# jake3991/sonar-SLAM

Measured on AMD Instinct MI355X. Metric: keyframes/sec (CFAR+ICP) on 512x1024 sonar, 5k-pt pairs, higher is better.
Workload: dtype u8 (CFAR, integer-exact) + f32/f64-accumulate (ICP); 1 GPU; BASELINE configs[1]: 4096 keyframes/step/GPU = 1024x512 SOCA-CFAR(Ntc40,Ngc10)+gate65 -> remap+nonzero+px2m -> downsample 0.5 -> remove_outlier 1.0/5 -> 5000x5000-pt ICP (p2plane30); batch_per_gpu=4096, distinct_frames=256, screened_out_pings=0, icp_mode=p2plane30, parallelism=job farm x1, icp_prep_stream=side, batches_in_flight=1, icp_converged_jobs=4096, max_points_per_frame=17494, points_capacity=32768, full=False

## Files before the change

### include/sonarfe.h

```cpp
#ifndef SONARFE_H
#define SONARFE_H

#include <stddef.h>
#include <stdint.h>

#ifdef __cplusplus
extern "C" {
#endif

typedef struct sfe_ctx sfe_ctx;
typedef struct sfe_geom sfe_geom;

#define SFE_ERR_ARG (-1)
#define SFE_ERR_HIP (-2)
#define SFE_ERR_NODEV (-3)
#define SFE_ERR_CAP (-4)

#define SFE_CFAR_CA 0
#define SFE_CFAR_SOCA 1
#define SFE_CFAR_GOCA 2
#define SFE_CFAR_OS 3

#define SFE_ICP_OK 0
#define SFE_ICP_NO_OUTLIER 1
// ... 119 lines not shown
int sfe_icp_compute_pairs_chain(sfe_ctx *ctx, const sfe_icp_params *p, const sfe_icp_dpf *rd, int n_rd,
                                const sfe_icp_dpf *rf, int n_rf, const float *src, const int32_t *src_off, const float *tgt,
                                const int32_t *tgt_off, const float *guesses9, int n_jobs, float *T_out9, int32_t *status,
                                int32_t *iters);
int sfe_icp_compute_jobs_chain(sfe_ctx *ctx, const sfe_icp_params *p, const sfe_icp_dpf *rd, int n_rd,
                               const sfe_icp_dpf *rf, int n_rf, const float *src, int n_src_pts, const float *tgt,
                               int n_tgt_pts, const int32_t *jobs4, const float *guesses9, int n_jobs, float *T_out9,
                               int32_t *status, int32_t *iters);
typedef struct sfe_icp_outliers {
    int use_min_dist;
    float min_dist;
    int use_median;
    float median_factor;
    int use_bound;
    float max_rotation_norm;
    float max_translation_norm;
    int bound_order;
} sfe_icp_outliers;
int sfe_icp_compute_guesses_chain_ext(sfe_ctx *ctx, const sfe_icp_params *p, const sfe_icp_outliers *o,
                                      const sfe_icp_dpf *rd, int n_rd, const sfe_icp_dpf *rf, int n_rf, const float *src,
                                      int n_src, const float *tgt, int n_tgt, const float *guesses9, int n_guesses,
                                      float *T_out9, int32_t *status, int32_t *iters);
int sfe_icp_compute_pairs_chain_ext(sfe_ctx *ctx, const sfe_icp_params *p, const sfe_icp_outliers *o,
                                    const sfe_icp_dpf *rd, int n_rd, const sfe_icp_dpf *rf, int n_rf, const float *src,
                                    const int32_t *src_off, const float *tgt, const int32_t *tgt_off, const float *guesses9,
                                    int n_jobs, float *T_out9, int32_t *status, int32_t *iters);
int sfe_icp_compute_jobs_chain_ext(sfe_ctx *ctx, const sfe_icp_params *p, const sfe_icp_outliers *o,
                                   const sfe_icp_dpf *rd, int n_rd, const sfe_icp_dpf *rf, int n_rf, const float *src,
                                   int n_src_pts, const float *tgt, int n_tgt_pts, const int32_t *jobs4, const float *guesses9,
                                   int n_jobs, float *T_out9, int32_t *status, int32_t *iters);
int sfe_icp_set_tuning(sfe_ctx *ctx, int variant);
int sfe_icp_get_profile(sfe_ctx *ctx, int enable, long long *cycles16);
#define SFE_ICP_ROUTE_TINY 0
#define SFE_ICP_ROUTE_T0 1
#define SFE_ICP_ROUTE_T1 2
#define SFE_ICP_ROUTE_Q 3
#define SFE_ICP_ROUTE_LDS 4
#define SFE_ICP_ROUTE_GLB 5
#define SFE_ICP_ROUTE_SPLIT 6
#define SFE_ICP_ROUTE_BRUTE 7
int sfe_icp_last_routes(sfe_ctx *ctx, int32_t *route, int n_jobs, int32_t *n_cu);
int sfe_icp_batch_dev(sfe_ctx *ctx, const sfe_icp_params *p, const float *d_src,
                      const int32_t *src_off, const float *d_tgt, const int32_t *tgt_off,
                      const float *d_guess9, int n_jobs, float *d_T9, int32_t *d_status,
                      int32_t *d_iters);

int sfe_icp_jobs_dev(sfe_ctx *ctx, const sfe_icp_params *p, const float *d_src, const float *d_tgt,
                     const int32_t *jobs4, const float *d_guess9, int n_jobs, float *d_T9, int32_t *d_status,
                     int32_t *d_iters);

int sfe_cloud_filter_batch_dev(sfe_ctx *ctx, const double *d_pts, const int32_t *d_counts, int n_frames,
                               int64_t cap, float resolution, double radius, int min_points,
                               float *d_out, int32_t *d_out_counts);
int sfe_cloud_filter_staged_dev(sfe_ctx *ctx, int n_frames, int64_t cap, float resolution, double radius,
                                int min_points, float *d_out, int32_t *d_out_counts);

int sfe_feature_extract_ping(sfe_ctx *ctx, sfe_geom *g, const uint8_t *img, int alg, int train_hs, int guard_hs,
                             int k, double tau, int intensity_thr, float resolution, double radius, int min_points,
                             int64_t cap, float *cloud_out, int32_t *n_out, int32_t *n_raw_out, uint8_t *vis_out);

typedef struct sfe_cloud_store sfe_cloud_store;
#define SFE_STORE_NEGATE_Y 1
#define SFE_PING_VIS_JET 4
#define SFE_STORE_F32_POINTS 2
int sfe_cloud_store_create(sfe_ctx *ctx, int64_t capacity_points, int32_t max_clouds, sfe_cloud_store **out);
void sfe_cloud_store_destroy(sfe_cloud_store *s);
int sfe_cloud_store_count(sfe_cloud_store *s);
int sfe_cloud_store_put(sfe_ctx *ctx, sfe_cloud_store *s, int64_t stamp, const float *pts, int n, int32_t *handle_out);
int sfe_cloud_store_put_batch_dev(sfe_ctx *ctx, sfe_cloud_store *s, const int64_t *stamps, const float *d_clouds,
                                  const int32_t *d_counts, int n_frames, int64_t cap, int flags, int32_t *handles_out);
int sfe_cloud_store_meta(sfe_ctx *ctx, sfe_cloud_store *s, int32_t first, int32_t n, int64_t *stamps, int64_t *offsets,
                         int32_t *counts);
int sfe_cloud_store_read(sfe_ctx *ctx, sfe_cloud_store *s, int32_t handle, float *out, int cap, int *n_out);
int sfe_cloud_store_truncate(sfe_ctx *ctx, sfe_cloud_store *s, int32_t n_slots);
int sfe_cloud_store_get_points(sfe_ctx *ctx, sfe_cloud_store *s, const int32_t *handles, const float *T6, int n_jobs, int m,
                               float resolution, int flags, const int64_t *stamps, int32_t *handles_out);
int sfe_icp_store_jobs_dev(sfe_ctx *ctx, const sfe_icp_params *p, sfe_cloud_store *s, const int32_t *pairs,
                           const float *d_guess9, int n_jobs, float *d_T9, int32_t *d_status, int32_t *d_iters);
int sfe_icp_store_compute(sfe_ctx *ctx, const sfe_icp_params *p, sfe_cloud_store *s, const int32_t *pairs,
                          const float *guesses9, int n_jobs, float *T_out9, int32_t *status, int32_t *iters);
int sfe_icp_store_compute_chain_ext(sfe_ctx *ctx, const sfe_icp_params *p, const sfe_icp_outliers *o,
                                    const sfe_icp_dpf *rd, int n_rd, const sfe_icp_dpf *rf, int n_rf,
                                    sfe_cloud_store *s, const int32_t *pairs, const float *guesses9, int n_jobs,
                                    float *T_out9, int32_t *status, int32_t *iters);
int sfe_cloud_store_overlap(sfe_ctx *ctx, sfe_cloud_store *s, const int32_t *pairs, const float *T6, int n_jobs,
                            float max_dist, int flags, int32_t *counts_out);
int sfe_cloud_store_get_points_keys(sfe_ctx *ctx, sfe_cloud_store *s, const int32_t *handles, const float *T6,
                                    const int32_t *keys, int m, float resolution, int flags, int64_t stamp, int32_t *handle_out);
int sfe_cloud_store_read_keys(sfe_ctx *ctx, sfe_cloud_store *s, int32_t handle, int32_t *out, int cap, int *n_out);
int sfe_cloud_store_fov_select(sfe_ctx *ctx, sfe_cloud_store *s, int32_t handle, const float *Tinv6, const double *range_bound,
                               const double *bearing_bound, int n_frames, int n_keys, int32_t *key_counts_out,
                               int32_t *n_selected_out, int32_t *n_ambiguous_out);
int sfe_cloud_store_set_selection(sfe_ctx *ctx, sfe_cloud_store *s, int32_t handle, const uint8_t *sel, int n);
int sfe_cloud_store_compact_selected(sfe_ctx *ctx, sfe_cloud_store *s, int32_t handle, int64_t stamp, int32_t *handle_out);
int sfe_cloud_store_match_keys(sfe_ctx *ctx, sfe_cloud_store *s, int32_t source, const float *T6, int32_t target, float max_dist,
                               int flags, int n_keys, int32_t *key_counts_out, int32_t *overlap_out);
int sfe_cloud_store_get_points_keys_many(sfe_ctx *ctx, sfe_cloud_store *s, const int32_t *handles, const float *T6,
                                         const int32_t *keys, const int32_t *job_off, int n_jobs, float resolution, int flags,
                                         const int64_t *stamps, int32_t *handles_out);
int sfe_cloud_store_fov_select_many(sfe_ctx *ctx, sfe_cloud_store *s, const int32_t *handles, int n_jobs, const float *Tinv6,
                                    const double *range_bound, const double *bearing_bound, const int32_t *frame_off,
                                    int n_keys, int32_t *key_counts_out, int32_t *n_selected_out, int32_t *n_ambiguous_out);
int sfe_cloud_store_compact_selected_many(sfe_ctx *ctx, sfe_cloud_store *s, const int32_t *handles, int n_jobs,
                                          const int64_t *stamps, int32_t *handles_out);
int sfe_cloud_store_match_keys_many(sfe_ctx *ctx, sfe_cloud_store *s, const int32_t *sources, const float *T6,
                                    const int32_t *targets, int n_jobs, float max_dist, int flags, int n_keys,
// ... 64 lines not shown
```

### sonar_slam_amd/_lib.py

```python
import contextlib
import ctypes as C
import os
import threading

import numpy as np

_HERE = os.path.dirname(os.path.abspath(__file__))
LIB_PATH = os.environ.get("SONARFE_LIB") or os.path.join(_HERE, "libsonarfe.so")

SFE_ERR_CAP = -4

ICP_ROUTE_TINY = 0
ICP_ROUTE_T0 = 1
ICP_ROUTE_T1 = 2
ICP_ROUTE_Q = 3
ICP_ROUTE_LDS = 4
ICP_ROUTE_GLB = 5
ICP_ROUTE_SPLIT = 6
ICP_ROUTE_BRUTE = 7

ALG = {"CA": 0, "SOCA": 1, "GOCA": 2, "OS": 3}

ICP_STATUS_MESSAGES = {
    0: "success",
# ... 124 lines not shown
    "sfe_geom_destroy": (None, [_vp]),
    "sfe_remap_u8": (C.c_int, [_vp, _vp, _u8p, _u8p]),
    "sfe_remap_u8_dev": (C.c_int, [_vp, _vp, _vp, _vp]),
    "sfe_colormap_lut": (C.c_int, [C.c_int, _u8p]),
    "sfe_remap_u8_colormap": (C.c_int, [_vp, _vp, _u8p, C.c_int, _u8p]),
    "sfe_remap_u8_colormap_dev": (C.c_int, [_vp, _vp, _vp, C.c_int, _vp]),
    "sfe_feature_extract_ping": (C.c_int, [_vp, _vp, _u8p, C.c_int, C.c_int, C.c_int, C.c_int, C.c_double, C.c_int, C.c_float,
                                           C.c_double, C.c_int, C.c_int64, _f32p, _i32p, _i32p, _u8p]),
    "sfe_extract_points": (C.c_int, [_vp, _vp, _u8p, C.c_int64, _i64p, _f64p, _i64p]),
    "sfe_extract_set_tuning": (C.c_int, [_vp, C.c_int]),
    "sfe_extract_points_batch_dev": (C.c_int, [_vp, _vp, _vp, C.c_int, C.c_int64, _vp, _vp]),
    "sfe_extract_points_bits_batch_dev": (C.c_int, [_vp, _vp, _vp, C.c_int, C.c_int64, _vp, _vp]),
    "sfe_extract_points_bits_staged_dev": (C.c_int, [_vp, _vp, _vp, C.c_int, C.c_int64, _vp, C.c_int, _vp]),
    "sfe_match": (C.c_int, [_vp, _f32p, C.c_int, _f32p, C.c_int, C.c_float, _i32p, _f32p]),
    "sfe_match_knn": (C.c_int, [_vp, _f32p, C.c_int, _f32p, C.c_int, C.c_int, C.c_float, _i32p, _f32p]),
    "sfe_knn_density": (C.c_int, [_vp, _f32p, C.c_int, C.c_int, _f32p]),
    "sfe_remove_outlier": (C.c_int, [_vp, _f32p, C.c_int, C.c_double, C.c_int, _f32p,
                                     C.POINTER(C.c_int)]),
    "sfe_downsample": (C.c_int, [_vp, _f32p, C.c_int, C.c_float, _f32p, _i32p, C.POINTER(C.c_int)]),
    "sfe_icp_compute": (C.c_int, [_vp, C.POINTER(IcpParams), _f32p, C.c_int, _f32p, C.c_int, _f32p,
                                  _f32p, C.POINTER(C.c_int)]),
    "sfe_icp_compute_guesses": (C.c_int, [_vp, C.POINTER(IcpParams), _f32p, C.c_int, _f32p, C.c_int,
                                          _f32p, C.c_int, _f32p, _i32p, _i32p]),
    "sfe_icp_compute_pairs": (C.c_int, [_vp, C.POINTER(IcpParams), _f32p, _i32p, _f32p, _i32p, _f32p, C.c_int,
                                        _f32p, _i32p, _i32p]),
    "sfe_icp_compute_jobs": (C.c_int, [_vp, C.POINTER(IcpParams), _f32p, C.c_int, _f32p, C.c_int, _i32p, _f32p, C.c_int,
                                       _f32p, _i32p, _i32p]),
    "sfe_icp_filter_clouds_dev": (C.c_int, [_vp, C.POINTER(IcpDpf), C.c_int, _vp, _i32p, C.c_int, _vp, _i32p]),
    "sfe_icp_compute_guesses_chain": (C.c_int, [_vp, C.POINTER(IcpParams), C.POINTER(IcpDpf), C.c_int, C.POINTER(IcpDpf),
                                                C.c_int, _f32p, C.c_int, _f32p, C.c_int, _f32p, C.c_int, _f32p, _i32p, _i32p]),
    "sfe_icp_compute_pairs_chain": (C.c_int, [_vp, C.POINTER(IcpParams), C.POINTER(IcpDpf), C.c_int, C.POINTER(IcpDpf),
                                              C.c_int, _f32p, _i32p, _f32p, _i32p, _f32p, C.c_int, _f32p, _i32p, _i32p]),
    "sfe_icp_compute_jobs_chain": (C.c_int, [_vp, C.POINTER(IcpParams), C.POINTER(IcpDpf), C.c_int, C.POINTER(IcpDpf),
                                             C.c_int, _f32p, C.c_int, _f32p, C.c_int, _i32p, _f32p, C.c_int, _f32p, _i32p,
                                             _i32p]),
    "sfe_icp_compute_guesses_chain_ext": (C.c_int, [_vp, C.POINTER(IcpParams), C.POINTER(IcpOutliers), C.POINTER(IcpDpf),
                                                    C.c_int, C.POINTER(IcpDpf), C.c_int, _f32p, C.c_int, _f32p, C.c_int,
                                                    _f32p, C.c_int, _f32p, _i32p, _i32p]),
    "sfe_icp_compute_pairs_chain_ext": (C.c_int, [_vp, C.POINTER(IcpParams), C.POINTER(IcpOutliers), C.POINTER(IcpDpf),
                                                  C.c_int, C.POINTER(IcpDpf), C.c_int, _f32p, _i32p, _f32p, _i32p, _f32p,
                                                  C.c_int, _f32p, _i32p, _i32p]),
    "sfe_icp_compute_jobs_chain_ext": (C.c_int, [_vp, C.POINTER(IcpParams), C.POINTER(IcpOutliers), C.POINTER(IcpDpf),
                                                 C.c_int, C.POINTER(IcpDpf), C.c_int, _f32p, C.c_int, _f32p, C.c_int, _i32p,
                                                 _f32p, C.c_int, _f32p, _i32p, _i32p]),
    "sfe_icp_set_tuning": (C.c_int, [_vp, C.c_int]),
    "sfe_icp_get_profile": (C.c_int, [_vp, C.c_int, C.POINTER(C.c_longlong)]),
    "sfe_icp_last_routes": (C.c_int, [_vp, _i32p, C.c_int, _i32p]),
    "sfe_icp_batch_dev": (C.c_int, [_vp, C.POINTER(IcpParams), _vp, _i32p, _vp, _i32p, _vp, C.c_int,
                                    _vp, _vp, _vp]),
    "sfe_icp_jobs_dev": (C.c_int, [_vp, C.POINTER(IcpParams), _vp, _vp, _i32p, _vp, C.c_int, _vp, _vp, _vp]),
    "sfe_cloud_filter_batch_dev": (C.c_int, [_vp, _vp, _vp, C.c_int, C.c_int64, C.c_float, C.c_double, C.c_int,
                                             _vp, _vp]),
    "sfe_cloud_filter_staged_dev": (C.c_int, [_vp, C.c_int, C.c_int64, C.c_float, C.c_double, C.c_int, _vp, _vp]),
    "sfe_cloud_store_create": (C.c_int, [_vp, C.c_int64, C.c_int32, C.POINTER(_vp)]),
    "sfe_cloud_store_destroy": (None, [_vp]),
    "sfe_cloud_store_count": (C.c_int, [_vp]),
    "sfe_cloud_store_put": (C.c_int, [_vp, _vp, C.c_int64, _f32p, C.c_int, _i32p]),
    "sfe_cloud_store_put_batch_dev": (C.c_int, [_vp, _vp, _i64p, _vp, _vp, C.c_int, C.c_int64, C.c_int, _i32p]),
    "sfe_cloud_store_meta": (C.c_int, [_vp, _vp, C.c_int32, C.c_int32, _i64p, _i64p, _i32p]),
    "sfe_cloud_store_read": (C.c_int, [_vp, _vp, C.c_int32, _f32p, C.c_int, C.POINTER(C.c_int)]),
    "sfe_cloud_store_truncate": (C.c_int, [_vp, _vp, C.c_int32]),
    "sfe_cloud_store_get_points": (C.c_int, [_vp, _vp, _i32p, _f32p, C.c_int, C.c_int, C.c_float, C.c_int, _i64p, _i32p]),
    "sfe_icp_store_jobs_dev": (C.c_int, [_vp, C.POINTER(IcpParams), _vp, _i32p, _vp, C.c_int, _vp, _vp, _vp]),
    "sfe_icp_store_compute": (C.c_int, [_vp, C.POINTER(IcpParams), _vp, _i32p, _f32p, C.c_int, _f32p, _i32p, _i32p]),
    "sfe_icp_store_compute_chain_ext": (C.c_int, [_vp, C.POINTER(IcpParams), C.POINTER(IcpOutliers), C.POINTER(IcpDpf),
                                                  C.c_int, C.POINTER(IcpDpf), C.c_int, _vp, _i32p, _f32p, C.c_int, _f32p,
                                                  _i32p, _i32p]),
    "sfe_cloud_store_overlap": (C.c_int, [_vp, _vp, _i32p, _f32p, C.c_int, C.c_float, C.c_int, _i32p]),
    "sfe_feature_extract_ping_store": (C.c_int, [_vp, _vp, _vp, C.c_int64, _u8p, C.c_int, C.c_int, C.c_int, C.c_int,
                                                 C.c_double, C.c_int, C.c_float, C.c_double, C.c_int, C.c_int64, C.c_int,
                                                 _i32p, _i32p, _i32p, _f32p, _u8p]),
    "sfe_costgrid_create": (C.c_int, [_vp, _i32p, _i32p, C.c_int, C.c_int, C.c_int, C.c_int, C.POINTER(_vp)]),
    "sfe_costgrid_destroy": (None, [_vp]),
    "sfe_costgrid_download": (C.c_int, [_vp, _vp, C.c_int, _u8p]),
    "sfe_matching_cost_batch": (C.c_int, [_vp, _vp, _f32p, C.c_int, _f32p, C.c_int, C.c_float, C.c_float,
                                          C.c_double, C.c_int, _i32p]),
    "sfe_costgrid_create_store": (C.c_int, [_vp, _vp, _i32p, C.c_int, _f32p, _f32p, C.c_float, _i32p, _i32p, C.c_int,
                                            C.POINTER(_vp)]),
    "sfe_matching_cost_store": (C.c_int, [_vp, _vp, _vp, _i32p, _i32p, C.c_int, _f32p, C.c_int, C.c_double, C.c_int, _i32p]),
    "sfe_shgo_sobol_replay": (C.c_int, [C.c_int, _i32p, _i32p, _f64p, _i32p, C.c_int, _u8p, _i32p, _i32p, _i32p]),
    "sfe_matching_cost_store_samples": (C.c_int, [_vp, _vp, _vp, _i32p, _i32p, C.c_int, _f64p, _f64p, _f64p, C.c_int, C.c_double, C.c_int,
                                                  _i32p]),
    "sfe_pose2_sample_transforms": (C.c_int, [_f64p, _f64p, C.c_int, _f64p, C.c_int, _f32p]),
    "sfe_cloud_store_bbox": (C.c_int, [_vp, _vp, _i32p, C.c_int, _f32p]),
    "sfe_cloud_store_get_points_keys": (C.c_int, [_vp, _vp, _i32p, _f32p, _i32p, C.c_int, C.c_float, C.c_int, C.c_int64, _i32p]),
    "sfe_cloud_store_read_keys": (C.c_int, [_vp, _vp, C.c_int32, _i32p, C.c_int, C.POINTER(C.c_int)]),
    "sfe_cloud_store_fov_select": (C.c_int, [_vp, _vp, C.c_int32, _f32p, _f64p, _f64p, C.c_int, C.c_int, _i32p, _i32p, _i32p]),
    "sfe_cloud_store_set_selection": (C.c_int, [_vp, _vp, C.c_int32, _u8p, C.c_int]),
    "sfe_cloud_store_compact_selected": (C.c_int, [_vp, _vp, C.c_int32, C.c_int64, _i32p]),
    "sfe_cloud_store_match_keys": (C.c_int, [_vp, _vp, C.c_int32, _f32p, C.c_int32, C.c_float, C.c_int, C.c_int, _i32p, _i32p]),
    "sfe_cloud_store_get_points_keys_many": (C.c_int, [_vp, _vp, _i32p, _f32p, _i32p, _i32p, C.c_int, C.c_float, C.c_int, _i64p,
                                                       _i32p]),
    "sfe_cloud_store_fov_select_many": (C.c_int, [_vp, _vp, _i32p, C.c_int, _f32p, _f64p, _f64p, _i32p, C.c_int, _i32p, _i32p,
                                                  _i32p]),
    "sfe_cloud_store_compact_selected_many": (C.c_int, [_vp, _vp, _i32p, C.c_int, _i64p, _i32p]),
    "sfe_cloud_store_match_keys_many": (C.c_int, [_vp, _vp, _i32p, _f32p, _i32p, C.c_int, C.c_float, C.c_int, C.c_int, _i32p,
                                                  _i32p]),
    "sfe_map_create": (C.c_int, [_vp, C.c_int, C.c_int, C.POINTER(_vp)]),
    "sfe_map_destroy": (None, [_vp]),
    "sfe_map_geometry": (C.c_int, [_vp, _f32p, C.c_int, C.c_int, C.POINTER(C.c_int)]),
    "sfe_map_set_logodds": (C.c_int, [_vp, C.c_int, C.c_int, _f32p]),
    "sfe_map_measure": (C.c_int, [_vp, C.c_int, _i32p, _i32p, _i32p, _i32p, _i32p, _i32p, _f32p, C.c_int, _f64p,
                                  C.c_float, C.c_float, C.c_float, C.c_float]),
    "sfe_map_measure_stages": (C.c_int, [_vp, C.c_int, _u8p, _f32p, _i32p]),
    "sfe_map_fit_bounds": (C.c_int, [_vp, C.c_int, _i32p, _f64p, _f64p, C.c_double, _i32p]),
    "sfe_map_grow": (C.c_int, [_vp, C.c_int, C.c_int, C.c_int, C.c_int]),
# ... 195 lines not shown
```

### sonar_slam_amd/csrc/sfe_cloudfilter.hip

```cpp
#include "sfe_cloudfilter.h"

#include <algorithm>
#include <cstdio>
#include <cstdlib>

__global__ __launch_bounds__(1024) void cf_cast_bbox_kernel(const double *__restrict__ pts64,
                                                            const int32_t *__restrict__ counts, long long cap,
                                                            float max_size, float2 *__restrict__ p32,
                                                            CfHeader *__restrict__ hdrs)
{
    __shared__ float s_mn[2][16], s_mx[2][16];
    const int f = blockIdx.x;
    const int n = (int)min((long long)max(counts[f], 0), cap);
    const double *src = pts64 + (size_t)f * cap * 2;
    float2 *dst = p32 + (size_t)f * cap;
    float mnx = INFINITY, mny = INFINITY, mxx = -INFINITY, mxy = -INFINITY;
    for (int i = threadIdx.x; i < n; i += 1024) {
        const float2 p = make_float2((float)src[2 * i], (float)src[2 * i + 1]);
        dst[i] = p;
        mnx = fminf(mnx, p.x);
        mxx = fmaxf(mxx, p.x);
        mny = fminf(mny, p.y);
        mxy = fmaxf(mxy, p.y);
    }
#pragma unroll
    for (int d = 32; d >= 1; d >>= 1) {
        mnx = fminf(mnx, __shfl_down(mnx, d));
        mxx = fmaxf(mxx, __shfl_down(mxx, d));
        mny = fminf(mny, __shfl_down(mny, d));
        mxy = fmaxf(mxy, __shfl_down(mxy, d));
    }
    if ((threadIdx.x & 63) == 0) {
        s_mn[0][threadIdx.x >> 6] = mnx;
        s_mn[1][threadIdx.x >> 6] = mny;
        s_mx[0][threadIdx.x >> 6] = mxx;
        s_mx[1][threadIdx.x >> 6] = mxy;
    }
    __syncthreads();
    if (threadIdx.x == 0) {
        for (int w = 1; w < 16; ++w) {
            mnx = fminf(mnx, s_mn[0][w]);
            mny = fminf(mny, s_mn[1][w]);
            mxx = fmaxf(mxx, s_mx[0][w]);
            mxy = fmaxf(mxy, s_mx[1][w]);
        }
        const CfHeader h = cf_make_header(mnx, mny, mxx, mxy, max_size, n);
        hdrs[f] = h;
    }
}

__device__ __forceinline__ unsigned long long cf_path_key(float2 p, const CfHeader &h)
{
    float cx = h.cx, cy = h.cy, r = h.radius;
    unsigned long long key = 0;
    for (int l = 0; l < h.levels; ++l) {
// ... 126 lines not shown
                                                             CfHeader *__restrict__ hdrs, float2 *__restrict__ ds_out,
                                                             int *__restrict__ seg_all, K *__restrict__ gkeys_all,
                                                             long long n2cap, int only_marked,
                                                             unsigned *__restrict__ leaf_keys_all, int *marked, int *n_marked,
                                                             const int *__restrict__ frame_list)
{
    if (frame_list) {
        const int nl = *n_marked;
        for (int i = blockIdx.x; i < nl; i += gridDim.x) {
            cf_downsample_frame<IN_LDS, K>(frame_list[i], blockIdx.x, p32, cap, hdrs, ds_out, seg_all, gkeys_all, n2cap, only_marked,
                                           leaf_keys_all, nullptr, nullptr);
            __syncthreads();
        }
    } else {
        cf_downsample_frame<IN_LDS, K>(blockIdx.x, blockIdx.x, p32, cap, hdrs, ds_out, seg_all, gkeys_all, n2cap, only_marked,
                                       leaf_keys_all, marked, n_marked);
    }
}

__device__ __forceinline__ int cf_block_excl_scan(int v, int *s_tmp, int *total)
{
    const int lane = threadIdx.x & 63, wave = threadIdx.x >> 6;
    int incl = v;
#pragma unroll
    for (int d = 1; d < 64; d <<= 1) {
        const int t = __shfl_up(incl, d);
        if (lane >= d)
            incl += t;
    }
    __syncthreads();
    if (lane == 63)
        s_tmp[wave] = incl;
    __syncthreads();
    if (wave == 0) {
        const int w = lane < 16 ? s_tmp[lane] : 0;
        int wi = w;
#pragma unroll
        for (int d = 1; d < 16; d <<= 1) {
            const int t = __shfl_up(wi, d);
            if (lane >= d)
                wi += t;
        }
        if (lane < 16)
            s_tmp[lane] = wi - w;
        if (lane == 15)
            s_tmp[16] = wi;
    }
    __syncthreads();
    *total = s_tmp[16];
    return incl - v + s_tmp[wave];
}

#define CF_RDX_BITS 4
#define CF_RDX_DIGITS (1 << CF_RDX_BITS)
#define CF_RDX_CHUNK 17
#define CF_RDX_CHUNK_BIG 19
#define CF_LDS_PTS_BIG (CF_RDX_CHUNK_BIG * 1024)
template <int CHUNK>
__global__ __launch_bounds__(1024) void cf_downsample_radix_kernel(const float2 *__restrict__ p32, long long cap,
                                                                   CfHeader *__restrict__ hdrs, float2 *__restrict__ ds_out,
                                                                   int *__restrict__ seg_all, int n2cap,
                                                                   unsigned *__restrict__ leaf_keys_all,
                                                                   float2 *__restrict__ spts_all, int lds_bytes, int sort_cols,
                                                                   int *marked, int *n_marked)
{
    extern __shared__ __attribute__((aligned(16))) unsigned char lds_raw[];
    __shared__ int s_scan[1024];
    const int f = blockIdx.x, tid = threadIdx.x;
    const CfHeader h = hdrs[f];
    const int n = h.n;
    const float2 *pts = p32 + (size_t)f * cap;
    float2 *out = ds_out + (size_t)f * cap;
    if (n == 0)
        return;
    if (n > n2cap) {
        if (tid == 0)
            cf_mark_global(hdrs, f, marked, n_marked);
        return;
    }
    if (2 * h.levels > 16) {
        if (tid == 0)
            hdrs[f].n_seg = CF_NEEDS_WIDE;
        return;
    }
    unsigned short *idA = reinterpret_cast<unsigned short *>(lds_raw);
    unsigned short *idB = idA + n2cap;
    unsigned short *skey = idB + n2cap;
    unsigned short *cnt = skey + n2cap;
    for (int i = tid; i < n; i += 1024) {
        idA[i] = (unsigned short)i;
        skey[i] = (unsigned short)cf_path_key(pts[i], h);
    }
    const int m = ((n + sort_cols - 1) / sort_cols) | 1;
    const bool col = tid < sort_cols;
    const int p0 = col ? min(tid * m, n) : n, p1 = min(p0 + m, n);
    const int passes = (2 * h.levels + CF_RDX_BITS - 1) / CF_RDX_BITS;
    if (col)
#pragma unroll
        for (int d = 0; d < CF_RDX_DIGITS; ++d) {
            const int f0 = d * sort_cols + tid;
            cnt[f0 + (f0 >> 4)] = 0;
        }
    auto slot = [&](int f) { return f + (f >> 4); };
    for (int pass = 0; pass < passes; ++pass) {
        const int shift = CF_RDX_BITS * pass;
        __syncthreads();
        unsigned id[CHUNK], dg[CHUNK];
#pragma unroll
        for (int k = 0; k < CHUNK; ++k)
            id[k] = p0 + k < p1 ? idA[p0 + k] : 0u;
#pragma unroll
        for (int k = 0; k < CHUNK; ++k)
            dg[k] = p0 + k < p1 ? ((unsigned)skey[id[k]] >> shift) & (CF_RDX_DIGITS - 1) : 0u;
#pragma unroll
        for (int k = 0; k < CHUNK; ++k)
            if (p0 + k < p1)
                cnt[slot(dg[k] * sort_cols + tid)] += 1;
        __syncthreads();
        {
            const int per_t = CF_RDX_DIGITS * sort_cols / 1024;
            const int base = slot(per_t * tid);
            int v[16], sum = 0;
#pragma unroll
            for (int k = 0; k < 16; ++k) {
                v[k] = k < per_t ? cnt[base + k] : 0;
                sum += v[k];
            }
            int tot_;
            int run = cf_block_excl_scan(sum, s_scan, &tot_);
#pragma unroll
            for (int k = 0; k < 16; ++k)
                if (k < per_t) {
                    cnt[base + k] = (unsigned short)run;
                    run += v[k];
                }
        }
        __syncthreads();
#pragma unroll
        for (int k = 0; k < CHUNK; ++k)
            if (p0 + k < p1) {
                const unsigned a = slot(dg[k] * sort_cols + tid);
                const unsigned off = cnt[a];
                idB[off] = (unsigned short)id[k];
                cnt[a] = (unsigned short)(off + 1);
            }
        if (col && pass + 1 < passes)
#pragma unroll
            for (int d = 0; d < CF_RDX_DIGITS; ++d)
                cnt[slot(d * sort_cols + tid)] = 0;
        unsigned short *t_ = idA;
        idA = idB;
        idB = t_;
    }
    __syncthreads();
    const int per = (n + 1023) / 1024;
    const int b0 = tid * per, e0 = min(b0 + per, n);
    int c = 0;
    {
        unsigned prev = (b0 > 0 && b0 < n) ? skey[idA[b0 - 1]] : 0u;
        for (int r = b0; r < e0; ++r) {
            const unsigned k = skey[idA[r]];
            c += (r == 0) || (k != prev);
            prev = k;
        }
    }
    int n_seg;
    const int seg_base = cf_block_excl_scan(c, s_scan, &n_seg);
    int *s_seg = seg_all + (size_t)f * (cap + 1);
    float2 *spts_g = spts_all + (size_t)f * cap;
    const bool in_lds = (size_t)n * sizeof(float2) <= (size_t)lds_bytes;
    {
        int sidx = seg_base;
        unsigned prev = (b0 > 0 && b0 < n) ? skey[idA[b0 - 1]] : 0u;
        for (int r = b0; r < e0; ++r) {
            const unsigned k = skey[idA[r]];
            if ((r == 0) || (k != prev))
                s_seg[sidx++] = r;
            prev = k;
        }
    }
    if (tid == 0)
        s_seg[n_seg] = n;
    __syncthreads();
    if (leaf_keys_all) {
        for (int sg = tid; sg < n_seg; sg += 1024)
            leaf_keys_all[(size_t)f * cap + sg] = (unsigned)skey[idA[s_seg[sg]]];
    }
    {
        constexpr int NV = CHUNK == CF_RDX_CHUNK ? 16 : CHUNK;
        float2 v[NV];
#pragma unroll
        for (int k = 0; k < NV; ++k) {
            const int r = tid + k * 1024;
            v[k] = r < n ? pts[idA[r]] : make_float2(0.0f, 0.0f);
        }
        __syncthreads();
        float2 *dst = in_lds ? reinterpret_cast<float2 *>(lds_raw) : spts_g;
#pragma unroll
        for (int k = 0; k < NV; ++k) {
            const int r = tid + k * 1024;
            if (r < n)
                dst[r] = v[k];
        }
    }
    __syncthreads();
    auto medoids = [&](const auto *spts) {
        for (int sg = tid; sg < n_seg; sg += 1024) {
            const int r0 = s_seg[sg], r1 = s_seg[sg + 1];
            float sx = 0.0f, sy = 0.0f;
            for (int r = r0; r < r1; ++r) {
                const float2 p = spts[r];
                sx = __fadd_rn(sx, p.x);
                sy = __fadd_rn(sy, p.y);
            }
            const float cntf = (float)(r1 - r0);
            sx = __fdiv_rn(sx, cntf);
            sy = __fdiv_rn(sy, cntf);
            float best = 3.402823466e+38f;
            int bi = r0;
            for (int r = r0; r < r1; ++r) {
                const float2 p = spts[r];
                const float dx = __fadd_rn(p.x, -sx), dy = __fadd_rn(p.y, -sy);
                const float d = sqrtf(__fadd_rn(__fmul_rn(dx, dx), __fmul_rn(dy, dy)));
                if (d < best) {
                    best = d;
                    bi = r;
                }
            }
            out[sg] = spts[bi];
        }
    };
    if (in_lds)
        medoids(reinterpret_cast<const float2 *>(lds_raw));
    else
        medoids(static_cast<const float2 *>(spts_g));
    if (tid == 0) {
        hdrs[f].n_seg = n_seg;
        hdrs[f].n_out = n_seg;
        hdrs[f].zlev = leaf_keys_all ? h.levels : -1;
    }
}

#define CF_CELL_LEVELS 6
#define CF_CELL_PTS 8192
__device__ __forceinline__ unsigned cf_spread(unsigned v)
{
    v = (v | (v << 4)) & 0x30Fu;
    v = (v | (v << 2)) & 0x333u;
    v = (v | (v << 1)) & 0x555u;
    return v;
}
__device__ __forceinline__ unsigned cf_squeeze(unsigned v)
{
    v &= 0x555u;
    v = (v | (v >> 1)) & 0x333u;
    v = (v | (v >> 2)) & 0x30Fu;
    v = (v | (v >> 4)) & 0x03Fu;
    return v;
}

__global__ __launch_bounds__(1024) void cf_radius_filter_kernel(const float2 *__restrict__ in_all, long long cap,
                                                                CfHeader *__restrict__ hdrs, float r2, int min_points,
                                                                float *__restrict__ out_all,
                                                                int32_t *__restrict__ out_counts, int do_filter,
                                                                const unsigned *__restrict__ leaf_keys_all)
{
    extern __shared__ __attribute__((aligned(16))) unsigned char cf_dyn[];
    float2 *s_p = reinterpret_cast<float2 *>(cf_dyn);
    __shared__ int s_scan[1024];
    const int f = blockIdx.x, tid = threadIdx.x;
    const CfHeader h = hdrs[f];
    const int n = h.n_seg;
    const float2 *pts = in_all + (size_t)f * cap;
    float2 *out = reinterpret_cast<float2 *>(out_all) + (size_t)f * cap;
    if (n < 0) {
        if (tid == 0)
            out_counts[f] = -1;
        return;
    }
    int lc = -1;
    if (do_filter && leaf_keys_all && h.zlev >= 0 && n <= CF_CELL_PTS && n > 0) {
        const float need = sqrtf(r2) * 1.001f;
        float width = h.radius * 2.0f;
        if (need > 0.0f && width >= need) {
            lc = 0;
            while (lc < CF_CELL_LEVELS && lc < h.zlev && width * 0.5f >= need) {
                width *= 0.5f;
                ++lc;
            }
        }
    }
    float2 *c_p = reinterpret_cast<float2 *>(cf_dyn);
    unsigned short *c_start = reinterpret_cast<unsigned short *>(cf_dyn + sizeof(float2) * CF_CELL_PTS);
// ... 105 lines not shown
    ctx->staged_frames = -1;
    float2 *d_p32 = (float2 *)sfe_scratch(ctx, CF_SLOT_P32, sizeof(float2) * per * (size_t)n_frames);
    CfHeader *d_hdr = (CfHeader *)sfe_scratch(ctx, CF_SLOT_HDR, sizeof(CfHeader) * (size_t)n_frames);
    if (!d_p32 || !d_hdr)
        return SFE_ERR_HIP;
    hipLaunchKernelGGL(cf_cast_bbox_kernel, dim3(n_frames), dim3(1024), 0, ctx->stream, d_pts, d_counts, (long long)cap,
                       sfe_cf_max_size(resolution), d_p32, d_hdr);
    return sfe_cf_run_staged(ctx, n_frames, cap, resolution, radius, min_points, d_out, d_out_counts);
}

extern "C" int sfe_cloud_filter_staged_dev(sfe_ctx *ctx, int n_frames, int64_t cap, float resolution, double radius, int min_points,
                                           float *d_out, int32_t *d_out_counts)
{
    if (int rc = sfe_use(ctx))
        return rc;
    SFE_ARG(ctx, n_frames >= 0 && cap > 0 && (n_frames == 0 || (d_out && d_out_counts)));
    if (ctx->staged_frames != n_frames || ctx->staged_cap != (long long)cap)
        return sfe_set_err(ctx, SFE_ERR_ARG, "sfe_cloud_filter_staged_dev: no staged clouds of %d frames x %lld points on this context "
                           "(sfe_extract_points_bits_staged_dev must precede it; found %d x %lld)", n_frames, (long long)cap,
                           ctx->staged_frames, ctx->staged_cap);
    if (n_frames == 0)
        return 0;
    CfBBox *d_bbox = (CfBBox *)sfe_scratch(ctx, CF_SLOT_BBOX, sizeof(CfBBox) * (size_t)n_frames);
    CfHeader *d_hdr = (CfHeader *)sfe_scratch(ctx, CF_SLOT_HDR, sizeof(CfHeader) * (size_t)n_frames);
    if (!d_bbox || !d_hdr)
        return SFE_ERR_HIP;
    hipLaunchKernelGGL(cf_header_from_bbox_kernel, dim3((unsigned)((n_frames + 255) / 256)), dim3(256), 0, ctx->stream,
                       (const CfBBox *)d_bbox, n_frames, sfe_cf_max_size(resolution), d_hdr);
    return sfe_cf_run_staged(ctx, n_frames, cap, resolution, radius, min_points, d_out, d_out_counts);
}

int sfe_cf_run_staged(sfe_ctx *ctx, int n_frames, int64_t cap, float resolution, double radius, int min_points,
                      float *d_out, int32_t *d_out_counts)
{
    const bool do_ds = resolution > 0.0f;
    const bool do_filter = min_points > 1;
    if (do_ds && cap > CF_MAX_CAP)
        return sfe_set_err(ctx, SFE_ERR_ARG, "resident cloud filter: cap %lld exceeds %d points per frame",
                           (long long)cap, CF_MAX_CAP);
    const size_t per = (size_t)std::max<int64_t>(cap, 1);
    float2 *d_p32 = (float2 *)sfe_scratch(ctx, CF_SLOT_P32, sizeof(float2) * per * (size_t)n_frames);
    float2 *d_ds = (float2 *)sfe_scratch(ctx, 26, sizeof(float2) * per * (size_t)n_frames);
    CfHeader *d_hdr = (CfHeader *)sfe_scratch(ctx, CF_SLOT_HDR, sizeof(CfHeader) * (size_t)n_frames);
    if (!d_p32 || !d_ds || !d_hdr)
        return SFE_ERR_HIP;
    const float2 *stage = d_p32;
    unsigned *d_lkeys = nullptr;
    if (do_ds) {
        size_t n2 = 2;
        while (n2 < (size_t)cap)
            n2 <<= 1;
        int *d_seg = (int *)sfe_scratch(ctx, 28, sizeof(int) * (per + 1) * (size_t)n_frames);
        d_lkeys = (unsigned *)sfe_scratch(ctx, 31, sizeof(unsigned) * per * (size_t)n_frames);
        float2 *d_spts = (float2 *)sfe_scratch(ctx, 40, sizeof(float2) * per * (size_t)n_frames);
        if (!d_seg || !d_lkeys || !d_spts)
            return SFE_ERR_HIP;
        {
            const size_t n2l = std::min<size_t>(n2, CF_SORT_CAP);
            const size_t n2r = cap <= CF_SORT_CAP ? n2 : (size_t)CF_LDS_PTS_BIG;
            int *d_marked = nullptr;
            if (cap > CF_SORT_CAP) {
                d_marked = (int *)sfe_scratch(ctx, 52, sizeof(int) * ((size_t)n_frames + 1));
                if (!d_marked)
                    return SFE_ERR_HIP;
                SFE_HIP(ctx, hipMemsetAsync(d_marked + n_frames, 0, sizeof(int), ctx->stream));
            }
            {
                const int sort_cols = n2r <= 8192 ? 512 : 1024;
                const size_t n_cnt = CF_RDX_DIGITS * (size_t)sort_cols;
                const bool big = n2r > CF_SORT_CAP;
                const size_t rdx_smem = big ? 3 * 2 * n2r + 2 * (n_cnt + n_cnt / 16)
                                            : std::max<size_t>(3 * 2 * n2r + 2 * (n_cnt + n_cnt / 16), sizeof(float2) * n2r);
                auto rk = big ? cf_downsample_radix_kernel<CF_RDX_CHUNK_BIG> : cf_downsample_radix_kernel<CF_RDX_CHUNK>;
                SFE_HIP(ctx, hipFuncSetAttribute((const void *)rk, hipFuncAttributeMaxDynamicSharedMemorySize, (int)rdx_smem));
                hipLaunchKernelGGL(rk, dim3(n_frames), dim3(1024), rdx_smem, ctx->stream, d_p32,
                                   (long long)cap, d_hdr, d_ds, d_seg, (int)n2r, d_lkeys, d_spts, (int)rdx_smem, sort_cols, d_marked,
                                   d_marked ? d_marked + n_frames : nullptr);
            }
            SFE_HIP(ctx, hipFuncSetAttribute((const void *)cf_downsample_kernel<true, unsigned long long>,
                                             hipFuncAttributeMaxDynamicSharedMemorySize, (int)(8 * n2l)));
            hipLaunchKernelGGL((cf_downsample_kernel<true, unsigned long long>), dim3(n_frames), dim3(1024), 8 * n2l,
                               ctx->stream, d_p32, (long long)cap, d_hdr, d_ds, d_seg, (unsigned long long *)nullptr, (long long)n2l, 1,
                               (unsigned *)nullptr, d_marked, d_marked ? d_marked + n_frames : nullptr, (const int *)nullptr);
            if (cap > CF_SORT_CAP) {
                const int gw = std::min(n_frames, 256);
                unsigned long long *d_gk = (unsigned long long *)sfe_scratch(ctx, 29, 8 * n2 * (size_t)gw);
                if (!d_gk)
                    return SFE_ERR_HIP;
                hipLaunchKernelGGL((cf_downsample_kernel<false, unsigned long long>), dim3(gw), dim3(1024), 0,
                                   ctx->stream, d_p32, (long long)cap, d_hdr, d_ds, d_seg, d_gk, (long long)n2, 1,
                                   (unsigned *)nullptr, (int *)nullptr, d_marked + n_frames, (const int *)d_marked);
            }
        }
        stage = d_ds;
    }
    const size_t cell_smem = sizeof(float2) * CF_CELL_PTS + sizeof(unsigned short) * ((1 << (2 * CF_CELL_LEVELS)) + 2);
    SFE_HIP(ctx, hipFuncSetAttribute((const void *)cf_radius_filter_kernel, hipFuncAttributeMaxDynamicSharedMemorySize,
                                     (int)cell_smem));
    hipLaunchKernelGGL(cf_radius_filter_kernel, dim3(n_frames), dim3(1024),
                       d_lkeys ? cell_smem : sizeof(float2) * 2048, ctx->stream, stage,
                       (long long)cap, d_hdr, (float)(radius * radius), min_points, d_out, d_out_counts, do_filter ? 1 : 0,
                       (const unsigned *)d_lkeys);
    SFE_LAUNCH_CHECK(ctx);
    return 0;
}
```

Before: 142,300 keyframes/s.

## Use adaptive 5-bit radix passes and keep downsample medoid points in LDS

The downsample radix kernel now picks 5-bit digits when that cuts the pass count and the count table fits in LDS. It packs the digit with the index in one register, skips the identity index initialisation on the first pass, and sizes LDS arrays by the padded point count instead of the power-of-two capacity. The global spill buffer for sorted points is removed and medoids always read from LDS, with a fast path for single-point cells. A host plan query and optional timestamp instrumentation are added. The risks are larger count tables, more register pressure, and the 8-bit packing in the scan, which assumes small per-thread counts.

Measured after the change: 143,000 keyframes/s (median of 6 runs). About the same (+0.5%).

```diff
diff --git a/include/sonarfe.h b/include/sonarfe.h
--- a/include/sonarfe.h
+++ b/include/sonarfe.h
@@ -195,6 +195,7 @@
 int sfe_cloud_filter_batch_dev(sfe_ctx *ctx, const double *d_pts, const int32_t *d_counts, int n_frames,
                                int64_t cap, float resolution, double radius, int min_points,
                                float *d_out, int32_t *d_out_counts);
+int sfe_cloud_filter_plan(int64_t cap, int n, int levels, int *plan);
 int sfe_cloud_filter_staged_dev(sfe_ctx *ctx, int n_frames, int64_t cap, float resolution, double radius,
                                 int min_points, float *d_out, int32_t *d_out_counts);
 
diff --git a/sonar_slam_amd/_lib.py b/sonar_slam_amd/_lib.py
--- a/sonar_slam_amd/_lib.py
+++ b/sonar_slam_amd/_lib.py
@@ -200,6 +200,7 @@
     "sfe_cloud_filter_batch_dev": (C.c_int, [_vp, _vp, _vp, C.c_int, C.c_int64, C.c_float, C.c_double, C.c_int,
                                              _vp, _vp]),
     "sfe_cloud_filter_staged_dev": (C.c_int, [_vp, C.c_int, C.c_int64, C.c_float, C.c_double, C.c_int, _vp, _vp]),
+    "sfe_cloud_filter_plan": (C.c_int, [C.c_int64, C.c_int, C.c_int, _i32p]),
     "sfe_cloud_store_create": (C.c_int, [_vp, C.c_int64, C.c_int32, C.POINTER(_vp)]),
     "sfe_cloud_store_destroy": (None, [_vp]),
     "sfe_cloud_store_count": (C.c_int, [_vp]),
diff --git a/sonar_slam_amd/csrc/sfe_cloudfilter.hip b/sonar_slam_amd/csrc/sfe_cloudfilter.hip
--- a/sonar_slam_amd/csrc/sfe_cloudfilter.hip
+++ b/sonar_slam_amd/csrc/sfe_cloudfilter.hip
@@ -1,6 +1,7 @@
 #include "sfe_cloudfilter.h"
 
 #include <algorithm>
+#include <type_traits>
 #include <cstdio>
 #include <cstdlib>
 
@@ -233,20 +234,86 @@
 }
 
 #define CF_RDX_BITS 4
-#define CF_RDX_DIGITS (1 << CF_RDX_BITS)
+#define CF_RDX_BITS_WIDE 5
 #define CF_RDX_CHUNK 17
 #define CF_RDX_CHUNK_BIG 19
 #define CF_LDS_PTS_BIG (CF_RDX_CHUNK_BIG * 1024)
+#define CF_LDS_DYN_MAX (160 * 1024 - 256)
+
+__host__ __device__ __forceinline__ int cf_cnt_bytes(int bits, int sort_cols)
+{
+    const int c = (1 << bits) * sort_cols;
+    return 2 * (c + c / 16);
+}
+
+struct CfSortPlan {
+    int bits, passes;
+};
+__host__ __device__ __forceinline__ int cf_pad8(int n) { return (n + 7) & ~7; }
+__host__ __device__ __forceinline__ CfSortPlan cf_sort_plan(int n, int levels, int sort_cols, int lds_bytes)
+{
+    CfSortPlan p;
+    const int kb = 2 * levels;
+    const int p4 = (kb + CF_RDX_BITS - 1) / CF_RDX_BITS, p5 = (kb + CF_RDX_BITS_WIDE - 1) / CF_RDX_BITS_WIDE;
+    const bool wide = p5 < p4 && 6 * cf_pad8(n) + cf_cnt_bytes(CF_RDX_BITS_WIDE, sort_cols) <= lds_bytes;
+    p.bits = wide ? CF_RDX_BITS_WIDE : CF_RDX_BITS;
+    p.passes = wide ? p5 : p4;
+    if (p.passes < 1)
+        p.passes = 1;
+    return p;
+}
+
+struct CfRadixLaunch {
+    int n2r, sort_cols, lds_bytes;
+    bool big;
+};
+static CfRadixLaunch cf_radix_launch(int64_t cap)
+{
+    size_t n2 = 2;
+    while (n2 < (size_t)cap)
+        n2 <<= 1;
+    CfRadixLaunch l;
+    l.n2r = cap <= CF_SORT_CAP ? (int)n2 : CF_LDS_PTS_BIG;
+    l.big = l.n2r > CF_SORT_CAP;
+    l.sort_cols = l.n2r <= 8192 ? 512 : 1024;
+    const int sort_b = 6 * l.n2r + cf_cnt_bytes(CF_RDX_BITS, l.sort_cols);
+    const int leaf_b = 8 * l.n2r;
+    l.lds_bytes = l.n2r > 8192 ? CF_LDS_DYN_MAX : std::max(sort_b, leaf_b);
+    return l;
+}
+
+#ifdef CF_STAMPS
+__device__ long long cf_stamps[16];
+__device__ int cf_stamp_frame;
+#define CF_STAMP(i)                                                                                                              \
+    do {                                                                                                                         \
+        if (threadIdx.x == 0 && (int)blockIdx.x == cf_stamp_frame)                                                               \
+            cf_stamps[i] = (long long)__builtin_amdgcn_s_memtime();                                                              \
+    } while (0)
+#define CF_STAMP_SYNC() __syncthreads()
+extern "C" int sfe_cf_stamps(int frame, long long *stamps)
+{
+    const long long zero[16] = {0};
+    if (hipDeviceSynchronize() != hipSuccess || hipMemcpyFromSymbol(stamps, HIP_SYMBOL(cf_stamps), sizeof zero) != hipSuccess ||
+        hipMemcpyToSymbol(HIP_SYMBOL(cf_stamps), zero, sizeof zero) != hipSuccess ||
+        hipMemcpyToSymbol(HIP_SYMBOL(cf_stamp_frame), &frame, sizeof frame) != hipSuccess)
+        return SFE_ERR_HIP;
+    return 0;
+}
+#else
+#define CF_STAMP(i)
+#define CF_STAMP_SYNC()
+#endif
+
 template <int CHUNK>
 __global__ __launch_bounds__(1024) void cf_downsample_radix_kernel(const float2 *__restrict__ p32, long long cap,
                                                                    CfHeader *__restrict__ hdrs, float2 *__restrict__ ds_out,
                                                                    int *__restrict__ seg_all, int n2cap,
-                                                                   unsigned *__restrict__ leaf_keys_all,
-                                                                   float2 *__restrict__ spts_all, int lds_bytes, int sort_cols,
+                                                                   unsigned *__restrict__ leaf_keys_all, int lds_bytes, int sort_cols,
                                                                    int *marked, int *n_marked)
 {
     extern __shared__ __attribute__((aligned(16))) unsigned char lds_raw[];
-    __shared__ int s_scan[1024];
+    __shared__ int s_scan[32];
     const int f = blockIdx.x, tid = threadIdx.x;
     const CfHeader h = hdrs[f];
     const int n = h.n;
@@ -264,76 +331,101 @@
             hdrs[f].n_seg = CF_NEEDS_WIDE;
         return;
     }
+    CF_STAMP(0);
+    const CfSortPlan plan = cf_sort_plan(n, h.levels, sort_cols, lds_bytes);
+    const int npad = cf_pad8(n);
     unsigned short *idA = reinterpret_cast<unsigned short *>(lds_raw);
-    unsigned short *idB = idA + n2cap;
-    unsigned short *skey = idB + n2cap;
-    unsigned short *cnt = skey + n2cap;
-    for (int i = tid; i < n; i += 1024) {
-        idA[i] = (unsigned short)i;
+    unsigned short *idB = idA + npad;
+    unsigned short *skey = idB + npad;
+    unsigned short *cnt = skey + npad;
+    for (int i = tid; i < n; i += 1024)
         skey[i] = (unsigned short)cf_path_key(pts[i], h);
-    }
     const int m = ((n + sort_cols - 1) / sort_cols) | 1;
     const bool col = tid < sort_cols;
     const int p0 = col ? min(tid * m, n) : n, p1 = min(p0 + m, n);
-    const int passes = (2 * h.levels + CF_RDX_BITS - 1) / CF_RDX_BITS;
-    if (col)
-#pragma unroll
-        for (int d = 0; d < CF_RDX_DIGITS; ++d) {
-            const int f0 = d * sort_cols + tid;
-            cnt[f0 + (f0 >> 4)] = 0;
-        }
-    auto slot = [&](int f) { return f + (f >> 4); };
-    for (int pass = 0; pass < passes; ++pass) {
-        const int shift = CF_RDX_BITS * pass;
-        __syncthreads();
-        unsigned id[CHUNK], dg[CHUNK];
-#pragma unroll
-        for (int k = 0; k < CHUNK; ++k)
-            id[k] = p0 + k < p1 ? idA[p0 + k] : 0u;
-#pragma unroll
-        for (int k = 0; k < CHUNK; ++k)
-            dg[k] = p0 + k < p1 ? ((unsigned)skey[id[k]] >> shift) & (CF_RDX_DIGITS - 1) : 0u;
-#pragma unroll
-        for (int k = 0; k < CHUNK; ++k)
-            if (p0 + k < p1)
-                cnt[slot(dg[k] * sort_cols + tid)] += 1;
-        __syncthreads();
-        {
-            const int per_t = CF_RDX_DIGITS * sort_cols / 1024;
-            const int base = slot(per_t * tid);
-            int v[16], sum = 0;
-#pragma unroll
-            for (int k = 0; k < 16; ++k) {
-                v[k] = k < per_t ? cnt[base + k] : 0;
-                sum += v[k];
-            }
-            int tot_;
-            int run = cf_block_excl_scan(sum, s_scan, &tot_);
-#pragma unroll
-            for (int k = 0; k < 16; ++k)
-                if (k < per_t) {
-                    cnt[base + k] = (unsigned short)run;
-                    run += v[k];
+    auto slot = [](int f) { return f + (f >> 4); };
+    auto sort = [&](auto width, auto columns) {
+        constexpr int BITS = decltype(width)::value, DIGITS = 1 << BITS, COLS = decltype(columns)::value;
+        constexpr int DSTRIDE = COLS + COLS / 16;
+        const int cbase = slot(tid);
+        if (col)
+#pragma unroll
+            for (int d = 0; d < DIGITS; ++d)
+                cnt[cbase + d * DSTRIDE] = 0;
+        for (int pass = 0; pass < plan.passes; ++pass) {
+            const int shift = BITS * pass;
+            __syncthreads();
+            CF_STAMP(1 + pass);
+            unsigned e[CHUNK];
+            if (pass == 0) {
+#pragma unroll
+                for (int k = 0; k < CHUNK; ++k)
+                    e[k] = (unsigned)(p0 + k) | (p0 + k < p1 ? ((unsigned)skey[p0 + k] & (DIGITS - 1)) << 16 : 0u);
+            } else {
+#pragma unroll
+                for (int k = 0; k < CHUNK; ++k)
+                    e[k] = p0 + k < p1 ? idA[p0 + k] : 0u;
+#pragma unroll
+                for (int k = 0; k < CHUNK; ++k)
+                    e[k] |= p0 + k < p1 ? (((unsigned)skey[e[k]] >> shift) & (DIGITS - 1)) << 16 : 0u;
+            }
+#pragma unroll
+            for (int k = 0; k < CHUNK; ++k)
+                if (p0 + k < p1)
+                    cnt[cbase + (e[k] >> 16) * DSTRIDE] += 1;
+            __syncthreads();
+            {
+                constexpr int per_t = DIGITS * COLS / 1024;
+                const int sbase = slot(per_t * tid);
+                unsigned v4[DIGITS / 4];
+                int sum = 0;
+#pragma unroll
+                for (int k = 0; k < DIGITS; ++k) {
+                    const unsigned v = k < per_t ? cnt[sbase + k + (per_t > 16 ? k >> 4 : 0)] : 0u;
+                    v4[k / 4] = (k % 4 ? v4[k / 4] : 0u) | (v << (8 * (k % 4)));
+                    sum += (int)v;
                 }
-        }
-        __syncthreads();
-#pragma unroll
-        for (int k = 0; k < CHUNK; ++k)
-            if (p0 + k < p1) {
-                const unsigned a = slot(dg[k] * sort_cols + tid);
-                const unsigned off = cnt[a];
-                idB[off] = (unsigned short)id[k];
-                cnt[a] = (unsigned short)(off + 1);
-            }
-        if (col && pass + 1 < passes)
-#pragma unroll
-            for (int d = 0; d < CF_RDX_DIGITS; ++d)
-                cnt[slot(d * sort_cols + tid)] = 0;
-        unsigned short *t_ = idA;
-        idA = idB;
-        idB = t_;
-    }
-    __syncthreads();
+                int tot_;
+                int run = cf_block_excl_scan(sum, s_scan, &tot_);
+#pragma unroll
+                for (int k = 0; k < DIGITS; ++k)
+                    if (k < per_t) {
+                        cnt[sbase + k + (per_t > 16 ? k >> 4 : 0)] = (unsigned short)run;
+                        run += (int)((v4[k / 4] >> (8 * (k % 4))) & 0xFFu);
+                    }
+            }
+            __syncthreads();
+#pragma unroll
+            for (int k = 0; k < CHUNK; ++k)
+                if (p0 + k < p1) {
+                    const unsigned a = cbase + (e[k] >> 16) * DSTRIDE;
+                    const unsigned off = cnt[a];
+                    idB[off] = (unsigned short)e[k];
+                    cnt[a] = (unsigned short)(off + 1);
+                }
+            if (col && pass + 1 < plan.passes)
+#pragma unroll
+                for (int d = 0; d < DIGITS; ++d)
+                    cnt[cbase + d * DSTRIDE] = 0;
+            unsigned short *t_ = idA;
+            idA = idB;
+            idB = t_;
+        }
+    };
+    using std::integral_constant;
+    if (plan.bits == CF_RDX_BITS_WIDE) {
+        if (sort_cols == 1024)
+            sort(integral_constant<int, CF_RDX_BITS_WIDE>(), integral_constant<int, 1024>());
+        else
+            sort(integral_constant<int, CF_RDX_BITS_WIDE>(), integral_constant<int, 512>());
+    } else {
+        if (sort_cols == 1024)
+            sort(integral_constant<int, CF_RDX_BITS>(), integral_constant<int, 1024>());
+        else
+            sort(integral_constant<int, CF_RDX_BITS>(), integral_constant<int, 512>());
+    }
+    __syncthreads();
+    CF_STAMP(1 + plan.passes);
     const int per = (n + 1023) / 1024;
     const int b0 = tid * per, e0 = min(b0 + per, n);
     int c = 0;
@@ -348,8 +440,6 @@
     int n_seg;
     const int seg_base = cf_block_excl_scan(c, s_scan, &n_seg);
     int *s_seg = seg_all + (size_t)f * (cap + 1);
-    float2 *spts_g = spts_all + (size_t)f * cap;
-    const bool in_lds = (size_t)n * sizeof(float2) <= (size_t)lds_bytes;
     {
         int sidx = seg_base;
         unsigned prev = (b0 > 0 && b0 < n) ? skey[idA[b0 - 1]] : 0u;
@@ -363,10 +453,12 @@
     if (tid == 0)
         s_seg[n_seg] = n;
     __syncthreads();
+    CF_STAMP(6);
     if (leaf_keys_all) {
         for (int sg = tid; sg < n_seg; sg += 1024)
             leaf_keys_all[(size_t)f * cap + sg] = (unsigned)skey[idA[s_seg[sg]]];
     }
+    float2 *spts = reinterpret_cast<float2 *>(lds_raw);
     {
         constexpr int NV = CHUNK == CF_RDX_CHUNK ? 16 : CHUNK;
         float2 v[NV];
@@ -376,50 +468,63 @@
             v[k] = r < n ? pts[idA[r]] : make_float2(0.0f, 0.0f);
         }
         __syncthreads();
-        float2 *dst = in_lds ? reinterpret_cast<float2 *>(lds_raw) : spts_g;
 #pragma unroll
         for (int k = 0; k < NV; ++k) {
             const int r = tid + k * 1024;
             if (r < n)
-                dst[r] = v[k];
-        }
-    }
-    __syncthreads();
-    auto medoids = [&](const auto *spts) {
-        for (int sg = tid; sg < n_seg; sg += 1024) {
-            const int r0 = s_seg[sg], r1 = s_seg[sg + 1];
-            float sx = 0.0f, sy = 0.0f;
-            for (int r = r0; r < r1; ++r) {
-                const float2 p = spts[r];
-                sx = __fadd_rn(sx, p.x);
-                sy = __fadd_rn(sy, p.y);
-            }
-            const float cntf = (float)(r1 - r0);
-            sx = __fdiv_rn(sx, cntf);
-            sy = __fdiv_rn(sy, cntf);
-            float best = 3.402823466e+38f;
-            int bi = r0;
-            for (int r = r0; r < r1; ++r) {
-                const float2 p = spts[r];
-                const float dx = __fadd_rn(p.x, -sx), dy = __fadd_rn(p.y, -sy);
-                const float d = sqrtf(__fadd_rn(__fmul_rn(dx, dx), __fmul_rn(dy, dy)));
-                if (d < best) {
-                    best = d;
-                    bi = r;
-                }
-            }
-            out[sg] = spts[bi];
-        }
-    };
-    if (in_lds)
-        medoids(reinterpret_cast<const float2 *>(lds_raw));
-    else
-        medoids(static_cast<const float2 *>(spts_g));
+                spts[r] = v[k];
+        }
+    }
+    __syncthreads();
+    CF_STAMP(7);
+    for (int sg = tid; sg < n_seg; sg += 1024) {
+        const int r0 = s_seg[sg], r1 = s_seg[sg + 1];
+        if (r1 - r0 == 1) {
+            out[sg] = spts[r0];
+            continue;
+        }
+        float sx = 0.0f, sy = 0.0f;
+        for (int r = r0; r < r1; ++r) {
+            const float2 p = spts[r];
+            sx = __fadd_rn(sx, p.x);
+            sy = __fadd_rn(sy, p.y);
+        }
+        const float cntf = (float)(r1 - r0);
+        sx = __fdiv_rn(sx, cntf);
+        sy = __fdiv_rn(sy, cntf);
+        float best = 3.402823466e+38f;
+        int bi = r0;
+        for (int r = r0; r < r1; ++r) {
+            const float2 p = spts[r];
+            const float dx = __fadd_rn(p.x, -sx), dy = __fadd_rn(p.y, -sy);
+            const float d = sqrtf(__fadd_rn(__fmul_rn(dx, dx), __fmul_rn(dy, dy)));
+            if (d < best) {
+                best = d;
+                bi = r;
+            }
+        }
+        out[sg] = spts[bi];
+    }
+    CF_STAMP_SYNC();
+    CF_STAMP(8);
     if (tid == 0) {
         hdrs[f].n_seg = n_seg;
         hdrs[f].n_out = n_seg;
         hdrs[f].zlev = leaf_keys_all ? h.levels : -1;
     }
+}
+
+extern "C" int sfe_cloud_filter_plan(int64_t cap, int n, int levels, int *plan)
+{
+    if (!plan || cap <= 0 || cap > CF_MAX_CAP || n < 0 || levels < 0)
+        return SFE_ERR_ARG;
+    const CfRadixLaunch l = cf_radix_launch(cap);
+    const CfSortPlan p = cf_sort_plan(n, levels, l.sort_cols, l.lds_bytes);
+    plan[0] = p.bits;
+    plan[1] = p.passes;
+    plan[2] = l.sort_cols;
+    plan[3] = n <= l.n2r && 2 * levels <= 16;
+    return 0;
 }
 
 #define CF_CELL_LEVELS 6
@@ -631,12 +736,11 @@
             n2 <<= 1;
         int *d_seg = (int *)sfe_scratch(ctx, 28, sizeof(int) * (per + 1) * (size_t)n_frames);
         d_lkeys = (unsigned *)sfe_scratch(ctx, 31, sizeof(unsigned) * per * (size_t)n_frames);
-        float2 *d_spts = (float2 *)sfe_scratch(ctx, 40, sizeof(float2) * per * (size_t)n_frames);
-        if (!d_seg || !d_lkeys || !d_spts)
+        if (!d_seg || !d_lkeys)
             return SFE_ERR_HIP;
         {
             const size_t n2l = std::min<size_t>(n2, CF_SORT_CAP);
-            const size_t n2r = cap <= CF_SORT_CAP ? n2 : (size_t)CF_LDS_PTS_BIG;
+            const CfRadixLaunch rl = cf_radix_launch(cap);
             int *d_marked = nullptr;
             if (cap > CF_SORT_CAP) {
                 d_marked = (int *)sfe_scratch(ctx, 52, sizeof(int) * ((size_t)n_frames + 1));
@@ -645,15 +749,10 @@
                 SFE_HIP(ctx, hipMemsetAsync(d_marked + n_frames, 0, sizeof(int), ctx->stream));
             }
             {
-                const int sort_cols = n2r <= 8192 ? 512 : 1024;
-                const size_t n_cnt = CF_RDX_DIGITS * (size_t)sort_cols;
-                const bool big = n2r > CF_SORT_CAP;
-                const size_t rdx_smem = big ? 3 * 2 * n2r + 2 * (n_cnt + n_cnt / 16)
-                                            : std::max<size_t>(3 * 2 * n2r + 2 * (n_cnt + n_cnt / 16), sizeof(float2) * n2r);
-                auto rk = big ? cf_downsample_radix_kernel<CF_RDX_CHUNK_BIG> : cf_downsample_radix_kernel<CF_RDX_CHUNK>;
-                SFE_HIP(ctx, hipFuncSetAttribute((const void *)rk, hipFuncAttributeMaxDynamicSharedMemorySize, (int)rdx_smem));
-                hipLaunchKernelGGL(rk, dim3(n_frames), dim3(1024), rdx_smem, ctx->stream, d_p32,
-                                   (long long)cap, d_hdr, d_ds, d_seg, (int)n2r, d_lkeys, d_spts, (int)rdx_smem, sort_cols, d_marked,
+                auto rk = rl.big ? cf_downsample_radix_kernel<CF_RDX_CHUNK_BIG> : cf_downsample_radix_kernel<CF_RDX_CHUNK>;
+                SFE_HIP(ctx, hipFuncSetAttribute((const void *)rk, hipFuncAttributeMaxDynamicSharedMemorySize, rl.lds_bytes));
+                hipLaunchKernelGGL(rk, dim3(n_frames), dim3(1024), (size_t)rl.lds_bytes, ctx->stream, d_p32,
+                                   (long long)cap, d_hdr, d_ds, d_seg, rl.n2r, d_lkeys, rl.lds_bytes, rl.sort_cols, d_marked,
                                    d_marked ? d_marked + n_frames : nullptr);
             }
             SFE_HIP(ctx, hipFuncSetAttribute((const void *)cf_downsample_kernel<true, unsigned long long>,
```
